# getreu/stringsext

Measured on AMD Instinct MI355X. Metric: GiB/s scanned, higher is better.
Workload: dtype u8

## Files before the change

### stringsext_amd/csrc/sx_api.cpp

```cpp
#include "sx_ctx.hpp"
#include "sx_print_core.hpp"
#include "sx_select_core.hpp"
#include "sx_selset_build.hpp"
#include "sx_selset_core.hpp"
#include "sx_selre_build.hpp"
#include "sx_selre_core.hpp"
#include "sx_extract_build.hpp"
#include "sx_extract_core.hpp"
#include "sx_seltally_build.hpp"
#include "sx_seltally_core.hpp"

using namespace sx;

struct sx_select_set {
    int device = 0;
    uint8_t* mem = nullptr;
    SelsetDevice dev{};
    sx_select_set_info info{};
};

struct sx_select_regex {
    int device = 0;
    uint8_t* mem = nullptr;
    SelreDevice dev{};
// ... 366 lines not shown
            if (d.d_pair_lut) (void)hipFree(d.d_pair_lut);
            if (d.d_wave_lut) (void)hipFree(d.d_wave_lut);
            if (d.d_wave_pairs) (void)hipFree(d.d_wave_pairs);
            if (d.d_wave_pairs2) (void)hipFree(d.d_wave_pairs2);
            for (void* q : d.d_rp) if (q) (void)hipFree(q);
            if (d.h_runs) (void)hipHostFree(d.h_runs);
            if (d.ev_runs) (void)hipEventDestroy(d.ev_runs);
            if (d.stream_w) (void)hipStreamDestroy(d.stream_w);
            if (d.h_tot) (void)hipHostFree(d.h_tot);
            if (d.h_small) (void)hipHostFree(d.h_small);
            for (hipEvent_t e : d.wave_ev) if (e) (void)hipEventDestroy(e);
            if (d.stream && d.stream != ctx->scan_stream) (void)hipStreamDestroy(d.stream);
        }
        for (int i = 0; i < 2; i++) {
            if (ctx->ing_pin[i]) (void)hipHostFree(ctx->ing_pin[i]);
            if (ctx->ing_dev[i]) (void)hipFree(ctx->ing_dev[i]);
        }
        if (ctx->copy_stream) (void)hipStreamDestroy(ctx->copy_stream);
        if (ctx->d2h_stream) (void)hipStreamDestroy(ctx->d2h_stream);
        if (ctx->scan_stream) (void)hipStreamDestroy(ctx->scan_stream);
        if (ctx->d_cache) (void)hipFree(ctx->d_cache);
        if (ctx->post_stream) (void)hipStreamDestroy(ctx->post_stream);
        if (ctx->merge_copy_stream) (void)hipStreamDestroy(ctx->merge_copy_stream);
        if (ctx->d_merge) (void)hipFree(ctx->d_merge);
        if (ctx->d_result) (void)hipFree(ctx->d_result);
        if (ctx->d_result_up) (void)hipFree(ctx->d_result_up);
        if (ctx->d_text) (void)hipFree(ctx->d_text);
        if (ctx->d_print_scratch) (void)hipFree(ctx->d_print_scratch);
        if (ctx->d_print_missions) (void)hipFree(ctx->d_print_missions);
        for (uint8_t* p : ctx->d_select) if (p) (void)hipFree(p);
        if (ctx->d_select_scratch) (void)hipFree(ctx->d_select_scratch);
        if (ctx->d_select_scratch2) (void)hipFree(ctx->d_select_scratch2);
        for (hipEvent_t e : ctx->merge_ev) if (e) (void)hipEventDestroy(e);
        if (ctx->ev_interleaved) (void)hipEventDestroy(ctx->ev_interleaved);
        if (ctx->d_input) (void)hipFree(ctx->d_input);
        if (ctx->d_scratch) (void)hipFree(ctx->d_scratch);
        if (ctx->h_pin) (void)hipHostFree(ctx->h_pin);
        if (ctx->h_pin2) (void)hipHostFree(ctx->h_pin2);
    }
    delete ctx;
}

const char* sx_last_error(const sx_ctx* ctx) { return ctx ? ctx->err.c_str() : g_create_error.c_str(); }

int sx_reset(sx_ctx* ctx) {
    if (!ctx) return SX_E_INVALID;
    for (size_t k = 0; k < ctx->missions.size(); k++) ctx->states[k].reset(ctx->missions[k]);
    ctx->shard_runs_valid = false;
    return SX_OK;
}


int sx_device_runs(sx_ctx* ctx, int mission_index, const void* device_bytes, uint64_t len, int stream_parity,
                   uint64_t min_chars, sx_run** runs, uint64_t* n_runs) {
    if (!ctx || !runs || !n_runs || mission_index < 0 || (size_t)mission_index >= ctx->missions.size()) return SX_E_INVALID;
    begin_call(ctx);
    ctx->sw.scan_warm = Switches::from_env().scan_warm;
    if (ctx->host_only) { ctx->err = "host-only context: no device scan"; return SX_E_STATE; }
    if ((uintptr_t)device_bytes & 15) { ctx->err = "device_bytes must be 16-byte aligned"; return SX_E_INVALID; }
    if (ctx->missions[(size_t)mission_index].host_sequential()) { ctx->err = "an ISO-2022-JP mission has no stage A (one sequential pass on the host)"; return SX_E_INVALID; }
    HIP_TRY(ctx, hipSetDevice(ctx->device));
    std::vector<RunList> out;
    ctx->shard_runs_valid = false;
    int rc = device_runs(ctx, { mission_index }, (const uint8_t*)device_bytes, len, { (uint32_t)(stream_parity & 1) },
                         { min_chars }, &out);
    if (rc != SX_OK) return rc;
// ... 699 lines not shown
```

### stringsext_amd/csrc/sx_ctx.hpp

```cpp
#pragma once
#include <hip/hip_runtime_api.h>
#include <stdio.h>
#include <stdlib.h>
#include <string.h>
#include <errno.h>
#include <fcntl.h>
#include <sys/mman.h>
#include <sys/stat.h>
#include <unistd.h>

#include <algorithm>
#include <atomic>
#include <chrono>
#include <condition_variable>
#include <deque>
#include <functional>
#include <mutex>
#include <string>
#include <thread>
#include <unordered_map>
#include <vector>

#include "sx_host.hpp"
#include "sx_switches.hpp"
// ... 52 lines not shown

struct ScanSlot {
    DevRun* d_recs = nullptr;
    uint32_t capacity = 0;
    uint32_t* d_counters = nullptr;
    hipEvent_t ev0 = nullptr, ev1 = nullptr;
    hipEvent_t ev_free = nullptr;
    bool free_pending = false;
    uint32_t* d_cnt = nullptr;  uint64_t cnt_cap = 0;
    uint32_t* d_grid = nullptr; uint64_t grid_cap = 0;
    DevRun* d_packed = nullptr; uint64_t packed_cap = 0;
    uint32_t region_cap = 0;
    uint64_t n_regions = 0;
    bool fused = false, fused_first = false;
};
struct MissionDev {
    hipStream_t stream = nullptr;
    hipStream_t stream_b = nullptr;
    ScanSlot slot[2];
    uint16_t* d_table = nullptr;
    uint32_t* d_pair_lut = nullptr;
    uint32_t* d_wave_pairs = nullptr;
    uint32_t* d_wave_pairs2 = nullptr;
    uint8_t* d_wave_lut = nullptr;
    sx_run* h_runs = nullptr; uint64_t h_runs_cap = 0;
    hipEvent_t ev_runs = nullptr;
    void* d_rp[12] = { nullptr, nullptr, nullptr, nullptr, nullptr, nullptr, nullptr, nullptr, nullptr, nullptr, nullptr, nullptr };
    uint64_t d_rp_cap[12] = { 0, 0, 0, 0, 0, 0, 0, 0, 0, 0, 0, 0 };
    hipStream_t stream_w = nullptr;
    uint64_t* h_tot = nullptr;
    const uint32_t* grid_of_scan = nullptr; uint32_t grid_sub = 0; const uint8_t* grid_data = nullptr; uint64_t grid_len = 0;
    uint8_t* h_small = nullptr;
    std::vector<hipEvent_t> wave_ev;
};


}

struct sx_result {
    sx::Result r;
};

struct sx_ctx {
    std::shared_ptr<sx::PinnedPool> pool = std::make_shared<sx::PinnedPool>();
    std::shared_ptr<std::atomic<uint64_t>> dev_epoch = std::make_shared<std::atomic<uint64_t>>(0);
    std::vector<sx::Mission> missions;
    std::vector<sx::ScannerState> states;
    std::vector<sx::MissionDev> dev;
    bool host_only = false;
    bool sharded_call = false, single_piece = true;
    int device = -1;
    sx_options opt{};
    sx::Switches sw;
    std::string err;
    sx_stats stats{};
    hipStream_t scan_stream = nullptr, post_stream = nullptr;
    uint8_t* d_cache = nullptr;
    uint64_t d_cache_cap = 0;
    hipStream_t merge_copy_stream = nullptr;
    hipEvent_t merge_ev[3] = { nullptr, nullptr, nullptr };
    uint8_t* d_merge = nullptr; uint64_t d_merge_cap = 0, merge_out_room = 0, merge_n_out = 0;
    uint8_t* d_result = nullptr; uint64_t d_result_cap = 0;
    uint8_t* d_result_up = nullptr; uint64_t d_result_up_cap = 0;
    uint8_t* d_text = nullptr; uint64_t d_text_cap = 0;
    uint8_t* d_print_scratch = nullptr; uint64_t d_print_scratch_cap = 0;
    uint8_t* d_print_missions = nullptr;
    uint8_t* d_select[2] = { nullptr, nullptr }; uint64_t d_select_cap[2] = { 0, 0 };
    std::shared_ptr<std::atomic<uint64_t>> select_epoch[2] = { std::make_shared<std::atomic<uint64_t>>(0), std::make_shared<std::atomic<uint64_t>>(0) };
    uint64_t select_calls = 0;
    uint8_t* d_select_scratch = nullptr; uint64_t d_select_scratch_cap = 0;
    uint8_t* d_select_scratch2 = nullptr; uint64_t d_select_scratch2_cap = 0;
    bool merge_async = false;
    bool merge_copy_pending[2] = { false, false };
    uint64_t merge_parts = 0;
    uint64_t merged_out_bytes = 0;
    double out_density = 0;
    hipEvent_t ev_interleaved = nullptr;
    std::atomic<bool> interleave_pending{ false };
    std::mutex mu;
    std::mutex err_mu;
    std::recursive_mutex grow_mu;
    void set_err(std::string text) { std::lock_guard<std::mutex> g(err_mu); err = std::move(text); }
    unsigned n_cus = 256, scan_blocks_per_cu = 8;
    hipStream_t copy_stream = nullptr;
    hipStream_t d2h_stream = nullptr;
    uint8_t* ing_pin[2] = { nullptr, nullptr };
    uint8_t* ing_dev[2] = { nullptr, nullptr };
    uint64_t ing_cap = 0, ing_dev_cap = 0;
    uint32_t region_cap = 64;
    std::vector<uint32_t> dense;
    uint8_t* d_input = nullptr;
    uint64_t d_input_cap = 0;
    uint64_t ondemand_fetches = 0;
// ... 68 lines not shown

private:
    struct Seg { uint64_t lo, hi; const uint8_t* p; };
    sx_ctx* ctx_;
    const uint8_t* d_base_;
    uint64_t len_ = 0;
    static constexpr uint64_t kBlock = 65536;
    std::unordered_map<uint64_t, std::vector<uint8_t>> blocks_;
    std::vector<Seg> segs_;
    std::deque<std::vector<uint8_t>> extra_, owned_;
    std::mutex mu_;
};

int ensure_pinned(sx_ctx* ctx, uint64_t bytes);
int ensure_pinned2(sx_ctx* ctx, uint64_t bytes);
int read_back_sync(sx_ctx* ctx, sx::MissionDev& d, hipStream_t s, void* host_dst, const void* dev_src, size_t bytes);
int read_back_async(sx_ctx* ctx, hipStream_t s, void* pinned_dst, const void* dev_src, size_t bytes);
int ensure_scratch(sx_ctx* ctx, uint64_t bytes);
int ensure_capacity(sx_ctx* ctx, ScanSlot& s, uint32_t cap);
int ensure_rp(sx_ctx* ctx, MissionDev& d, int slot, uint64_t bytes);
int ensure_cache(sx_ctx* ctx, uint64_t bytes);
unsigned usable_cpus();
unsigned replay_threads(const sx_ctx* ctx);
void begin_call(sx_ctx* ctx);

ScanParams scan_params(const sx_ctx* ctx, int mission, const ScanSlot& s, const uint8_t* d_bytes, uint64_t len,
                       uint32_t parity, uint64_t min_chars);
int stage_a_launch(sx_ctx* ctx, const std::vector<int>& which, const uint8_t* d_bytes, uint64_t len,
                   const std::vector<uint32_t>& parity, const std::vector<uint64_t>& min_chars, int si);
struct ReplayJob;
int ensure_copy_stream(sx_ctx* ctx);
bool result_stays_on_device(const sx_ctx* ctx, const ReplayJob& job);
int merge_drain(sx_ctx* ctx);
int stage_a_finish(sx_ctx* ctx, const std::vector<int>& which, const uint8_t* d_bytes, uint64_t len,
                   const std::vector<uint32_t>& parity, const std::vector<uint64_t>& min_chars, int si,
                   std::vector<RunList>* out, bool cut_into_pieces = false, const ReplayJob* wave_job = nullptr);
int device_runs(sx_ctx* ctx, const std::vector<int>& which, const uint8_t* d_bytes, uint64_t len,
                const std::vector<uint32_t>& parity, const std::vector<uint64_t>& min_chars,
                std::vector<RunList>* out);

struct ReplayJob {
    uint64_t len = 0;
    int file_id = -1;
    bool is_last = false;
    std::vector<uint64_t> lo;
    uint64_t hi = 0;
    std::vector<char> entry_exact;
    std::vector<uint64_t> consumed0, stream0;
    bool commit_state = true;
    uint32_t slice_base = 0;
    const uint8_t* d_bytes = nullptr;
};




struct PreReplayed {
    std::vector<char> done;
    std::vector<MissionFindings> per;
    std::vector<uint64_t> ends;
    explicit PreReplayed(size_t nm) : done(nm, 0), per(nm), ends(nm, 0) {}
};


constexpr int SX_WAVE_FALLBACK = 1001;
constexpr int SX_NEED_RUNS = 1002;
// ... 34 lines not shown
```

### stringsext_amd/csrc/sx_replay.cpp

```cpp
#include <stdio.h>
#include <string.h>

#include <algorithm>
#include <atomic>
#include <deque>
#include <mutex>
#include <thread>

#include "sx_host.hpp"
#include "sx_replay_core.hpp"

namespace sx {

static inline uint64_t window_start(uint64_t p, size_t W) {
    const uint64_t s = p / kInputBufLen * kInputBufLen;
    return s + (p - s) / W * W;
}
static inline uint64_t back_windows(uint64_t p, size_t W, int k) {
    uint64_t w = window_start(p, W);
    for (int i = 0; i < k && w > 0; i++) w = window_start(w - 1, W);
    return w;
}
static inline uint64_t window_end(uint64_t p, size_t W, uint64_t len) {
    const uint64_t s = p / kInputBufLen * kInputBufLen;
// ... 485 lines not shown
        while (open_end && k < v.size() && (v[k].chars_flags & kRecStartOpen) && v[k].start == r.end) {
            r.end = v[k].start + v[k].len;
            r.chars += v[k].chars_flags & kRecCharsMask;
            open_end = (v[k].chars_flags & kRecEndOpen) != 0;
            k++;
        }
        if (r.chars >= min_chars) out->push_back(r);
        i = k;
    }
}

void merge_sorted_device_runs(const DevRun* v, size_t n, uint64_t min_chars, std::vector<sx_run>* out) {
    out->clear();
    out->reserve(n / 2);
    for (size_t i = 0; i < n && v[i].start != ~0ull;) {
        sx_run r{ v[i].start, v[i].start + v[i].len, v[i].chars_flags & kRecCharsMask };
        bool open_end = (v[i].chars_flags & kRecEndOpen) != 0;
        size_t k = i + 1;
        while (open_end && k < n && v[k].start != ~0ull && (v[k].chars_flags & kRecStartOpen) && v[k].start == r.end) {
            r.end = v[k].start + v[k].len;
            r.chars += v[k].chars_flags & kRecCharsMask;
            open_end = (v[k].chars_flags & kRecEndOpen) != 0;
            k++;
        }
        if (r.chars >= min_chars) out->push_back(r);
        i = k;
    }
}

void merge_findings(std::vector<MissionFindings>& per, const std::shared_ptr<PinnedPool>& pool, Result* out, uint64_t seg_bytes) {
    out->pool = pool;
    size_t nonempty = 0, which = 0;
    for (size_t k = 0; k < per.size(); k++) if (per[k].count()) { nonempty++; which = k; }
    auto release = [&](MissionFindings& mf) { if (mf.ext.p && pool) pool->give(mf.ext); mf.ext = {}; };
    if (nonempty <= 1) {
        for (size_t k = 0; k < per.size(); k++) if (!(nonempty == 1 && k == which)) release(per[k]);
        if (nonempty == 1) {
            std::vector<MissionFindings> more = std::move(per[which].more);
            per[which].more.clear();
            out->segs.push_back(std::move(per[which])); per[which].ext = {};
            for (auto& m : more) { out->segs.push_back(std::move(m)); m.ext = {}; }
        }
        return;
    }
    size_t total = 0, bytes = 0;
    for (auto& mf : per) { total += mf.count(); bytes += mf.strings_len(); }
    std::vector<size_t> idx(per.size(), 0);
    const uint64_t seg_cap = seg_bytes ? seg_bytes : 0xFFFFFFF0ull;
    if (bytes <= seg_cap) {
        out->segs.emplace_back();
        MissionFindings& m = out->segs.back();
        m.v.reserve(total);
        m.arena.reserve(bytes);
        std::vector<size_t> base(per.size(), 0);
        for (size_t k = 0; k < per.size(); k++) { base[k] = m.arena.size(); m.arena.append(per[k].strings(), per[k].strings_len()); }
        for (;;) {
            int best = -1;
            for (size_t k = 0; k < per.size(); k++) {
                if (idx[k] >= per[k].count()) continue;
                if (best < 0) { best = (int)k; continue; }
                const sx_finding& a = per[k].data()[idx[k]];
                const sx_finding& b = per[best].data()[idx[best]];
                if (a.slice_index < b.slice_index || (a.slice_index == b.slice_index && a.position < b.position)) best = (int)k;
            }
            if (best < 0) break;
            sx_finding f = per[best].data()[idx[best]++];
            f.str_off += (uint32_t)base[best];
            m.v.push_back(f);
        }
        total = 0;
    }
    size_t done = 0;
    while (done < total) {
        out->segs.emplace_back();
        MissionFindings& m = out->segs.back();
        m.v.reserve(std::min<size_t>(total - done, 1u << 24));
        for (;;) {
            int best = -1;
            for (size_t k = 0; k < per.size(); k++) {
                if (idx[k] >= per[k].count()) continue;
                if (best < 0) { best = (int)k; continue; }
// ... 91 lines not shown
```

### stringsext_amd/csrc/sx_schedule.cpp

```cpp
#include "sx_ctx.hpp"
#include <thread>

using namespace sx;

namespace sx {

uint64_t piece_bytes(const sx_ctx* ctx, uint64_t len) {
    uint64_t piece = 0;
    bool halves = false;
    if (ctx->sw.piece_mib >= 0) piece = (uint64_t)ctx->sw.piece_mib << 20;
    else if (len >= (16ull << 30) && ctx->missions.size() >= 2 && !(ctx->opt.flags & (SX_OPT_NO_FUSED_SCAN | SX_OPT_MISSION_STREAMS | SX_OPT_RESULT_ON_DEVICE))) {
        piece = ((len / 100) * 50 + kInputBufLen - 1) / kInputBufLen * kInputBufLen;
        halves = true;
    }
    if (piece == 0 || (!halves && len < 2 * piece)) return len;
    for (const Mission& m : ctx->missions) if (m.is_dbcs()) return len;
    return piece / kInputBufLen * kInputBufLen;
}

static uint64_t seq_piece_bytes(const sx_ctx* ctx, uint64_t len) {
    uint64_t piece = 0;
    if (ctx->sw.seq_piece_kib >= 0) {
        piece = (uint64_t)ctx->sw.seq_piece_kib << 10;
        if (piece == 0) return len;
// ... 77 lines not shown
               && ctx->sw.wave_replay != 0;
    }
    bool none_scanned(const sx_ctx* ctx) const {
        if (not_scanned.size() != ctx->missions.size()) return false;
        for (char c : not_scanned) if (!c) return false;
        return true;
    }

    int fetch_base(sx_ctx* ctx) {
        base_view.reset();
        if (host_bytes) return SX_OK;
        base_view.reset(new SparseDeviceBytes(ctx, d_bytes, len));
        if (none_scanned(ctx)) return SX_OK;
        ReplayJob none;
        return download_for_replay(ctx, d_bytes, len, nullptr, base_view.get(), none);
    }
    std::vector<char> not_scanned;
    int launch(sx_ctx* ctx) {
        not_scanned.assign(ctx->missions.size(), 0);
        std::vector<int> ks; std::vector<uint32_t> par; std::vector<uint64_t> mc;
        for (int k : order) {
            if (ctx->missions[(size_t)k].host_sequential() || skip_scan(ctx, (size_t)k)) { not_scanned[(size_t)k] = 1; continue; }
            ks.push_back(k); par.push_back(parity[(size_t)k]); mc.push_back(minc[(size_t)k]);
        }
        return ks.empty() ? SX_OK : stage_a_launch(ctx, ks, d_bytes, len, par, mc, slot);
    }
    int finish_and_replay(sx_ctx* ctx, const ReplayJob& job, const std::function<int()>& after_last_finish,
                          std::vector<RunList>* runs, Result* into, uint64_t* ends) {
        const size_t nm = ctx->missions.size();
        runs->assign(nm, RunList{});
        HostBytes host_view(host_bytes ? host_bytes : (const uint8_t*)"");
        ByteView& early_view = host_bytes ? (ByteView&)host_view : (ByteView&)*base_view;
        PreReplayed pre(nm);
        if (ctx->last_runs.size() != nm) ctx->last_runs.assign(nm, 0);
        ctx->wave_off.assign(nm, 0);
        if (ctx->wave_pred.size() != nm) ctx->wave_pred.assign(nm, 0);
        std::vector<std::thread> wave_threads(nm);
        std::vector<int> wave_rc(nm, SX_OK);
        std::vector<char> threaded(nm, 0);
        struct Joiner {
            std::vector<std::thread>& t;
            ~Joiner() { for (auto& x : t) if (x.joinable()) x.join(); }
        } joiner{ wave_threads };
        const uint64_t defer_all = nm >= 2 ? (result_stays_on_device(ctx, job) ? 1 : ctx->sw.defer_min_bytes) : 0;
        if (nm >= 2 && ctx->sw.wave_threads) {
            if (ctx->wave_density.size() != nm) ctx->wave_density.assign(nm, 0.0);
            for (size_t k = 0; k < nm; k++) {
                const bool unscanned = k < not_scanned.size() && not_scanned[k];
                if (ctx->missions[k].host_sequential() || !unscanned || !wave_replay_wanted(ctx, job, k, len)) continue;
                threaded[k] = 1;
                ctx->stats.bytes_scanned += len;
                wave_threads[k] = std::thread([ctx, k, &early_view, &job, &pre, &wave_rc, defer_all]() {
                    (void)hipSetDevice(ctx->device);
                    wave_rc[k] = wave_replay_mission(ctx, k, early_view, job, &pre.per[k], &pre.ends[k], defer_all, true);
                });
            }
        }
        std::vector<size_t> order2;
        for (size_t oi = 0; oi < nm; oi++) if (!threaded[(size_t)order[oi]]) order2.push_back((size_t)order[oi]);
        for (size_t oi = 0; oi < nm; oi++) if (threaded[(size_t)order[oi]]) order2.push_back((size_t)order[oi]);
        for (size_t oi = 0; oi < nm; oi++) {
            const size_t k = order2[oi];
            std::vector<RunList> one;
            int rc = SX_OK;
            const bool unscanned = k < not_scanned.size() && not_scanned[k];
            bool replayed = false;
// ... 281 lines not shown
```

### stringsext_amd/csrc/sx_stage_b.cpp

```cpp
#include "sx_ctx.hpp"

using namespace sx;

namespace sx {

static inline uint64_t win_start_h(uint64_t p, size_t W) {
    const uint64_t s0 = p / kInputBufLen * kInputBufLen;
    return s0 + (p - s0) / W * W;
}

bool device_replay_wanted(const sx_ctx* ctx, const ReplayJob& job, size_t k, size_t n_runs) {
    if (!job.d_bytes || ctx->host_only || job.is_last || ctx->missions[k].host_sequential()) return false;
    if (ctx->opt.flags & SX_OPT_HOST_REPLAY) return false;
    if (ctx->missions[k].q > 255) return false;
    if (ctx->missions[k].c.chars_min_nb == 0) return false;
    if (ctx->sw.host_replay) return false;
    if (wave_replay_wanted(ctx, job, k, n_runs)) return true;
    return (ctx->opt.flags & SX_OPT_DEVICE_REPLAY) || ctx->sw.device_replay || n_runs >= 4096;
}

struct Slab {
    size_t i0 = 0, i1 = 0;
    bool first = true, last = true;
    int out_slot = 5;
    bool async_copy = false;
    hipEvent_t reuse_after = nullptr;
    hipEvent_t copied = nullptr;
    uint64_t lo0 = 0;
    bool entry_exact0 = false;
};
struct SlabCarry {
    uint64_t last_start = 0;
    bool last_is_entry = false, any = false;
};
constexpr int SX_RETRY_WHOLE = 1000;

static int device_replay_slab(sx_ctx* ctx, size_t k, ByteView& view, const ReplayJob& job, const RunList& runs, const Slab& sl,
                              SlabCarry& carry, MissionFindings* out, uint64_t* end_pos, uint64_t defer_min_bytes) {
    const Mission& m = ctx->missions[k];
    MissionDev& d = ctx->dev[k];
    const size_t n_all = runs.size();
    const size_t n = sl.i1 - sl.i0;
    const bool slabbed = !(sl.first && sl.last);
    const size_t W = m.window;
    const double t0 = now_ms();

    ReplayParams P{};
    bool fast_pass = false;
    bool dev_stitch = n > 0 && !ctx->sw.host_stitch;
    uint64_t* h_tot = nullptr;
    ReplayRegionOut* ro = nullptr;
    {
        int rc = ensure_pinned2(ctx, (dev_stitch ? 0 : n * sizeof(ReplayRegionOut)) + 512);
        if (rc != SX_OK) return rc;
        h_tot = (uint64_t*)ctx->h_pin2;
        ro = (ReplayRegionOut*)(ctx->h_pin2 + 384);
    }
    if (n) {
        int rc = ensure_rp(ctx, d, 0, n * sizeof(sx_run)); if (rc) return rc;
        rc = ensure_rp(ctx, d, 1, n * sizeof(ReplayRegionOut)); if (rc) return rc;
// ... 66 lines not shown
    if (dev_stitch) HIP_TRY(ctx, runs.fetch_edges(kEdgeRuns)); else HIP_TRY(ctx, runs.wait());
    const size_t head_n = runs.full() ? n_all : kEdgeRuns;
    std::deque<ReplayPart> host_parts;
    struct Seg { int host_part; size_t v0, v1; };
    std::vector<Seg> segs;
    uint64_t E = std::min(job.lo[k], job.hi);
    uint64_t last_start = carry.any ? carry.last_start : E;
    bool last_is_entry = carry.any ? carry.last_is_entry : false;
    if (job.entry_exact[k]) {
        host_parts.emplace_back();
        replay_part(m, ctx->states[k], job.consumed0[k], job.stream0[k], view, job.len, job.file_id, false, runs.data(), head_n,
                    job.lo[k], job.lo[k] + 1, true, &host_parts.back());
        if (head_n < n_all && host_parts.back().end_pos >= runs[head_n - 1].start) {
            HIP_TRY(ctx, runs.wait());
            host_parts.pop_back();
            host_parts.emplace_back();
            replay_part(m, ctx->states[k], job.consumed0[k], job.stream0[k], view, job.len, job.file_id, false, runs.data(), n_all,
                        job.lo[k], job.lo[k] + 1, true, &host_parts.back());
        }
        if (host_parts.back().regions.empty()) host_parts.pop_back();
        else { segs.push_back({ (int)host_parts.size() - 1, 0, 0 }); last_is_entry = true; E = std::max(E, host_parts.back().end_pos); }
        E = std::max(E, job.lo[k] + 1);
    }
    if (dev_stitch) {
        HIP_TRY(ctx, launch_stitch_finish(P, (const ReplayRegionOut*)d.d_rp[1], (uint8_t*)d.d_rp[2], d.d_rp[6], E,
                                          (uint64_t*)d.d_rp[3], (uint64_t*)d.d_rp[4], (uint64_t*)d.d_rp[7], ctx->d_scratch,
                                          ctx->d_scratch_cap, d.stream_b, ctx->sw.stitch_block));
        { const int rb = read_back_async(ctx, d.stream_b, h_tot, d.d_rp[7], kTotCount * 8); if (rb != SX_OK) return rb; }
    }
    SX_TL("  replay: pass 1 + stitch queued, host entry part done");
    if (n) HIP_TRY(ctx, hipStreamSynchronize(d.stream_b));
    SX_TL("  replay: pass 1 + stitch done");
    if (dev_stitch && h_tot[kTotTooLong] && slabbed) return SX_RETRY_WHOLE;
    if (dev_stitch && h_tot[kTotTooLong]) {
        dev_stitch = false;
        HIP_TRY(ctx, runs.wait());
        const uint64_t keep32 = h_tot[32], keep33 = h_tot[33];
        int rc = ensure_pinned2(ctx, n * sizeof(ReplayRegionOut) + 512);
        if (rc != SX_OK) return rc;
        h_tot = (uint64_t*)ctx->h_pin2;
        h_tot[32] = keep32; h_tot[33] = keep33;
        ro = (ReplayRegionOut*)(ctx->h_pin2 + 384);
        HIP_TRY(ctx, hipMemcpyAsync(ro, d.d_rp[1], n * sizeof(ReplayRegionOut), hipMemcpyDeviceToHost, d.stream_b));
        HIP_TRY(ctx, hipStreamSynchronize(d.stream_b));
    }
    const double t1 = now_ms();
    if (fast_pass && n) {
        std::lock_guard<std::mutex> g(ctx->mu);
        ctx->stats.fast_regions += (uint32_t)h_tot[33] - (uint32_t)h_tot[32];
        ctx->stats.general_regions += (uint32_t)h_tot[32];
    }

    std::vector<uint64_t> valid, fbase, abase;
    uint64_t nf = 0, nb = 0, n_standing = 0;
    if (dev_stitch) {
        nf = h_tot[kTotFindings]; nb = h_tot[kTotBytes]; n_standing = h_tot[kTotStanding];
        out->replay_bytes += h_tot[kTotReplayBytes];
        if (h_tot[kTotLast] != ~0ull) {
            E = std::max(E, h_tot[kTotEnd]);
            last_start = h_tot[kTotLastStart];
            last_is_entry = false;
        }
    } else {
        valid.reserve(n); fbase.reserve(n + 1); abase.reserve(n + 1);
        for (size_t i = 0; i < n; i++) {
            const uint32_t st = ro[i].status;
// ... 37 lines not shown
            else HIP_TRY(ctx, hipStreamWaitEvent(d.stream_b, sl.reuse_after, 0));
        }
        int rc = ensure_rp(ctx, d, sl.out_slot, out_bytes + 64); if (rc) return rc;
        uint8_t* d_all = (uint8_t*)d.d_rp[sl.out_slot];
        sx_finding* d_f = (sx_finding*)d_all + nfh;
        uint8_t* d_a = d_all + (nfh + nf) * sizeof(sx_finding) + nbh;
        if (dev_stitch) {
            P.str_off_base = (uint32_t)nbh;
            HIP_TRY(ctx, launch_replay_write_flagged(P, (const ReplayRegionOut*)d.d_rp[1], (const uint8_t*)d.d_rp[2],
                                                     (const uint64_t*)d.d_rp[3], (const uint64_t*)d.d_rp[4], d_f, d_a,
                                                     (nf * sizeof(sx_finding) + nb) / std::max<uint64_t>(1, n_standing), d.stream_b));
            if (nfh) {
                entry_f.assign(hf0->v.begin(), hf0->v.end());
                for (sx_finding& f : entry_f) f.slice_index += job.slice_base;
                HIP_TRY(ctx, hipMemcpyAsync(d_all, entry_f.data(), nfh * sizeof(sx_finding), hipMemcpyHostToDevice, d.stream_b));
                if (nbh) HIP_TRY(ctx, hipMemcpyAsync(d_all + (nfh + nf) * sizeof(sx_finding), hf0->arena.data(), nbh, hipMemcpyHostToDevice, d.stream_b));
            }
        } else {
            const size_t nv = valid.size();
            HIP_TRY(ctx, hipMemcpyAsync(d.d_rp[2], valid.data(), nv * 8, hipMemcpyHostToDevice, d.stream_b));
            HIP_TRY(ctx, hipMemcpyAsync(d.d_rp[3], fbase.data(), (nv + 1) * 8, hipMemcpyHostToDevice, d.stream_b));
            HIP_TRY(ctx, hipMemcpyAsync(d.d_rp[4], abase.data(), (nv + 1) * 8, hipMemcpyHostToDevice, d.stream_b));
            HIP_TRY(ctx, launch_replay_write(P, (const uint64_t*)d.d_rp[2], (const uint64_t*)d.d_rp[3],
                                             (const uint64_t*)d.d_rp[4], nv, d_f, d_a, d.stream_b));
        }
        deferred = defer_min_bytes && nf * sizeof(sx_finding) + nb >= defer_min_bytes && dev_stitch && (host_parts.empty() || entry_only);
        keep_dev = (ctx->opt.flags & SX_OPT_RESULT_ON_DEVICE) && ctx->missions.size() == 1 && defer_min_bytes == 0 && job.commit_state && !ctx->sharded_call &&
                   ctx->single_piece && sl.first && sl.last && !sl.async_copy && dev_stitch && (host_parts.empty() || entry_only);
        deferred = deferred || keep_dev;
        if (!deferred) {
            blk = ctx->pool->take(out_bytes + 64);
            if (!blk.p) { ctx->err = "hipHostMalloc failed"; return SX_E_NOMEM; }
            if (sl.async_copy) {
                HIP_TRY(ctx, hipEventRecord(ctx->merge_ev[0], d.stream_b));
                HIP_TRY(ctx, hipStreamWaitEvent(ctx->merge_copy_stream, ctx->merge_ev[0], 0));
                HIP_TRY(ctx, hipMemcpyAsync(blk.p, d_all, out_bytes, hipMemcpyDeviceToHost, ctx->merge_copy_stream));
                HIP_TRY(ctx, hipEventRecord(sl.copied, ctx->merge_copy_stream));
            } else {
                const int wgs = ctx->sw.replay_copy_wgs;
                if (wgs > 0 && out_bytes >= (1u << 20)) HIP_TRY(ctx, launch_copy_bytes(blk.p, d_all, out_bytes, (uint32_t)wgs, d.stream_b, ctx->sw.merge_copy_threads, ctx->sw.merge_copy_nt != 0));
                else HIP_TRY(ctx, hipMemcpyAsync(blk.p, d_all, out_bytes, hipMemcpyDeviceToHost, d.stream_b));
            }
        }
        SX_TL("  replay: pass 2 + copy queued (%llu bytes%s)", (unsigned long long)out_bytes, deferred ? ", stays on the device" : "");
        if (!sl.async_copy || nfh) HIP_TRY(ctx, hipStreamSynchronize(d.stream_b));
        SX_TL("  replay: pass 2 + copy done");
    }
    const double t3 = now_ms();

    if (host_parts.empty() || (entry_only && (blk.p || deferred))) {
        if (deferred) {
            out->dev_only = true; out->ext_nf = nfh + nf; out->ext_na = nbh + nb; out->dev_copy = d.d_rp[sl.out_slot];
            if (keep_dev) { out->keep_on_device = true; out->dev_epoch_ref = ctx->dev_epoch; out->dev_epoch = ctx->dev_epoch->load(); }
        }
        else if (blk.p) { out->ext = blk; out->ext_nf = nfh + nf; out->ext_na = nbh + nb; out->dev_copy = sl.async_copy ? nullptr : d.d_rp[sl.out_slot]; }
        if (hf0) out->replay_bytes += hf0->replay_bytes;
    } else {
        const sx_finding* dev_f = (const sx_finding*)blk.p;
        const char* dev_a = blk.p ? (const char*)blk.p + nf * sizeof(sx_finding) : nullptr;
        if (dev_stitch) {
            fbase.assign({ 0, nf }); abase.assign({ 0, nb });
            if (n_standing) segs.push_back({ -1, 0, 1 });
        }
        for (const Seg& g : segs) {
            if (g.host_part >= 0) {
                const MissionFindings& hf = host_parts[(size_t)g.host_part].findings;
                const uint32_t base = (uint32_t)out->arena.size();
                out->arena += hf.arena;
// ... 14 lines not shown
        uint64_t ts = win_start_h(tail, W);
        for (int t = 0; t < 3 && ts > 0; t++) ts = win_start_h(ts - 1, W);
        const uint64_t lo0 = slabbed ? sl.lo0 : job.lo[k];
        const bool exact0 = slabbed ? sl.entry_exact0 : job.entry_exact[k] != 0;
        uint64_t from = last_is_entry ? lo0 : (E > ts ? last_start : ts);
        if (from < lo0) from = lo0;
        ReplayPart fin;
        const sx_run* fr = runs.data();
        size_t fn = n_all;
        if (!runs.full()) {
            if (n_all > kEdgeRuns && runs[n_all - kEdgeRuns].start <= from) { fr = runs.data() + (n_all - kEdgeRuns); fn = kEdgeRuns; }
            else HIP_TRY(ctx, runs.wait());
        }
        replay_part(m, ctx->states[k], job.consumed0[k], job.stream0[k], view, job.len, job.file_id, false, fr, fn,
                    from, job.len, exact0 && from == lo0, &fin);
        ctx->states[k] = fin.state;
        ctx->states[k].consumed_bytes = job.consumed0[k] + job.len;
        ctx->states[k].stream_bytes = job.stream0[k] + job.len;
        E = job.len;
    }
    if (end_pos) *end_pos = std::max(E, std::min(job.hi, job.len));
    carry.last_start = last_start; carry.last_is_entry = last_is_entry; carry.any = true;
    if (ctx->sw.timing)
        fprintf(stderr, "[sx] device replay mission %zu: %zu runs, pass1+entry %.2f ms, validity %.2f ms (%zu standing, %zu host parts), "
                        "pass2+d2h %.2f ms (%llu findings), splice+state %.2f ms\n", k, n, t1 - t0, t2 - t1, (size_t)n_standing,
                host_parts.size(), t3 - t2, (unsigned long long)nf, now_ms() - t3);
    return SX_OK;
}

int ensure_copy_stream(sx_ctx* ctx) {
    if (ctx->merge_copy_stream) return SX_OK;
    HIP_TRY(ctx, hipStreamCreateWithPriority(&ctx->merge_copy_stream, hipStreamNonBlocking, 0));
    for (hipEvent_t& e : ctx->merge_ev) HIP_TRY(ctx, hipEventCreateWithFlags(&e, hipEventDisableTiming));
    return SX_OK;
}

int device_replay_mission(sx_ctx* ctx, size_t k, ByteView& view, const ReplayJob& job, const RunList& runs,
                          MissionFindings* out, uint64_t* end_pos, uint64_t defer_min_bytes) {
    const size_t n = runs.size();
    MissionDev& d = ctx->dev[k];
    if (wave_replay_wanted(ctx, job, k, n)) {
        const int rc = wave_replay_mission(ctx, k, view, job, out, end_pos, defer_min_bytes);
        if (rc != SX_WAVE_FALLBACK) return rc;
        if (k < ctx->wave_off.size()) ctx->wave_off[k] = 1;
        if (k < ctx->wave_pred.size()) ctx->wave_pred[k] = 0;
    }
    if (runs.skipped) return SX_NEED_RUNS;
    size_t K = 1;
    const bool can = ctx->missions.size() == 1 && runs.on_device && !ctx->sw.host_stitch && defer_min_bytes == 0;
    const bool keep_dev_wanted = (ctx->opt.flags & SX_OPT_RESULT_ON_DEVICE) && ctx->missions.size() == 1 && defer_min_bytes == 0 && job.commit_state && !ctx->sharded_call && ctx->single_piece;
    if (can && n >= (1u << 20) && !keep_dev_wanted) K = 3;
    if (ctx->sw.slabs) { K = (size_t)ctx->sw.slabs; if (!can || n < 8 * K) K = 1; }
    std::vector<uint64_t> idx{ 0 }, his{ 0 };
    if (K > 1) {
        int rc = ensure_copy_stream(ctx); if (rc != SX_OK) return rc;
        rc = ensure_scratch(ctx, 4096); if (rc != SX_OK) return rc;
        rc = ensure_pinned2(ctx, 4096); if (rc != SX_OK) return rc;
        ReplayParams P{};
        P.runs = runs.dev_ptr; P.n_runs = n; P.W = (uint32_t)ctx->missions[k].window; P.grep_char = ctx->missions[k].c.grep_char;
        uint64_t* d_cut = (uint64_t*)ctx->d_scratch;
        HIP_TRY(ctx, launch_slab_cuts(P, (uint32_t)K, d_cut, d_cut + 64, d.stream_b));
        { const int rb = read_back_async(ctx, d.stream_b, ctx->h_pin2, d_cut, 128 * 8); if (rb != SX_OK) return rb; }
        HIP_TRY(ctx, hipStreamSynchronize(d.stream_b));
        const uint64_t* h = (const uint64_t*)ctx->h_pin2;
        for (size_t j = 1; j < K; j++)
            if (h[j - 1] > idx.back() && h[j - 1] < n && h[64 + j - 1] < job.hi) { idx.push_back(h[j - 1]); his.push_back(h[64 + j - 1]); }
    }
    idx.push_back(n);
    const size_t ns = idx.size() - 1;
    if (ns > 1) {
        std::vector<MissionFindings> got;
        SlabCarry carry;
        hipEvent_t copied[2] = { ctx->merge_ev[1], ctx->merge_ev[2] };
        uint64_t e_prev = 0;
        int rc = SX_OK;
        for (size_t j = 0; j < ns && rc == SX_OK; j++) {
            ReplayJob sj = job;
            sj.hi = j + 1 < ns ? std::min(job.hi, his[j + 1]) : job.hi;
            if (j > 0) { sj.lo[k] = std::max(job.lo[k], e_prev); sj.entry_exact[k] = 0; }
            sj.commit_state = job.commit_state && j + 1 == ns;
            Slab sl;
            sl.i0 = idx[j]; sl.i1 = idx[j + 1]; sl.first = j == 0; sl.last = j + 1 == ns;
            sl.out_slot = (j & 1) ? 8 : 5; sl.async_copy = true;
            sl.reuse_after = j >= 2 ? copied[j & 1] : nullptr; sl.copied = copied[j & 1];
            sl.lo0 = job.lo[k]; sl.entry_exact0 = job.entry_exact[k] != 0;
            MissionFindings mf;
            uint64_t e_now = 0;
            rc = device_replay_slab(ctx, k, view, sj, runs, sl, carry, &mf, &e_now, 0);
            e_prev = std::max(e_prev, e_now);
            if (rc == SX_OK) {
                out->replay_bytes += mf.replay_bytes; mf.replay_bytes = 0;
                if (mf.count()) got.push_back(std::move(mf));
            } else if (mf.ext.p) got.push_back(std::move(mf));
        }
        (void)hipStreamSynchronize(ctx->merge_copy_stream);
        (void)hipStreamSynchronize(d.stream_b);
        if (rc == SX_OK) {
            const uint64_t rb = out->replay_bytes;
            if (!got.empty()) {
                *out = std::move(got[0]);
                for (size_t j = 1; j < got.size(); j++) out->more.push_back(std::move(got[j]));
            }
            out->replay_bytes = rb;
            if (end_pos) *end_pos = e_prev;
            return SX_OK;
        }
        for (auto& g : got) if (g.ext.p) ctx->pool->give(g.ext);
        out->replay_bytes = 0;
        if (rc != SX_RETRY_WHOLE) return rc;
    }
    Slab sl;
    sl.i1 = n;
    SlabCarry carry;
    return device_replay_slab(ctx, k, view, job, runs, sl, carry, out, end_pos, defer_min_bytes);
}

static int fetch_deferred(sx_ctx* ctx, MissionFindings& mf) {
    if (!mf.dev_only) return SX_OK;
    const size_t bytes = mf.ext_nf * sizeof(sx_finding) + mf.ext_na;
    PinnedPool::Block blk = ctx->pool->take(bytes + 64);
    if (!blk.p) { ctx->err = "hipHostMalloc failed"; return SX_E_NOMEM; }
    HIP_TRY(ctx, hipMemcpyAsync(blk.p, mf.dev_copy, bytes, hipMemcpyDeviceToHost, ctx->post_stream));
    HIP_TRY(ctx, hipStreamSynchronize(ctx->post_stream));
    mf.ext = blk; mf.dev_only = false;
    return SX_OK;
}

bool result_stays_on_device(const sx_ctx* ctx, const ReplayJob& job) {
    return (ctx->opt.flags & SX_OPT_RESULT_ON_DEVICE) && ctx->missions.size() >= 2 && merge_part_can_pack(1, (int)ctx->missions.size()) && !ctx->host_only &&
           job.d_bytes && job.commit_state && !ctx->sharded_call && ctx->single_piece && !ctx->sw.host_merge;
}

static int upload_host_lists(sx_ctx* ctx, std::vector<MissionFindings>& per, std::vector<char>& uploaded) {
    uint64_t need = 0;
    for (auto& mf : per) {
        if (!mf.count() || mf.dev_copy) continue;
        if (!mf.more.empty() || mf.packed) return SX_E_NOMEM;
        need += (mf.count() * sizeof(sx_finding) + mf.strings_len() + 255) & ~(uint64_t)255;
    }
    if (!need) return SX_OK;
    if (ctx->d_result_up_cap < need) {
        if (ctx->d_result_up) HIP_TRY(ctx, hipFree(ctx->d_result_up));
        ctx->d_result_up = nullptr; ctx->d_result_up_cap = 0;
        if (hipMalloc((void**)&ctx->d_result_up, need) != hipSuccess) { (void)hipGetLastError(); ctx->d_result_up = nullptr; return SX_E_NOMEM; }
        ctx->d_result_up_cap = need;
    }
    PinnedPool::Block blk = ctx->pool->take(need);
    if (!blk.p) return SX_E_NOMEM;
    uint64_t at = 0;
    for (size_t k = 0; k < per.size(); k++) {
        MissionFindings& mf = per[k];
        if (!mf.count() || mf.dev_copy) continue;
        const uint64_t fb = mf.count() * sizeof(sx_finding);
        memcpy((uint8_t*)blk.p + at, mf.data(), fb);
        memcpy((uint8_t*)blk.p + at + fb, mf.strings(), mf.strings_len());
        mf.dev_copy = ctx->d_result_up + at; uploaded[k] = 1;
        at += (fb + mf.strings_len() + 255) & ~(uint64_t)255;
    }
    hipError_t e = hipMemcpyAsync(ctx->d_result_up, blk.p, need, hipMemcpyHostToDevice, ctx->post_stream);
    if (e == hipSuccess) e = hipStreamSynchronize(ctx->post_stream);
    ctx->pool->give(blk);
    if (e != hipSuccess) {
        for (size_t k = 0; k < per.size(); k++) if (uploaded[k]) { per[k].dev_copy = nullptr; uploaded[k] = 0; }
        HIP_TRY(ctx, e);
    }
    return SX_OK;
}

int merge_drain(sx_ctx* ctx) {
    std::lock_guard<std::recursive_mutex> g(ctx->grow_mu);
    if (ctx->post_stream) HIP_TRY(ctx, hipStreamSynchronize(ctx->post_stream));
    if (ctx->merge_copy_stream) HIP_TRY(ctx, hipStreamSynchronize(ctx->merge_copy_stream));
    ctx->merge_copy_pending[0] = ctx->merge_copy_pending[1] = false;
    ctx->interleave_pending = false;
    return SX_OK;
}

static int device_merge(sx_ctx* ctx, const ReplayJob& job, std::vector<MissionFindings>& per, Result* into) {
    const size_t nm = per.size();
    size_t with = 0, on_dev = 0, deferred = 0;
    uint64_t total = 0, bytes = 0;
    bool same_origin = true;
    for (size_t k = 0; k < nm; k++) {
        if (!per[k].count()) continue;
        with++;
        if ((per[k].ext.p || per[k].dev_only) && per[k].dev_copy) on_dev++;
        if (per[k].dev_only) deferred++;
        total += per[k].count(); bytes += per[k].strings_len();
        same_origin = same_origin && job.consumed0[k] == job.consumed0[0];
    }
    std::vector<char> uploaded(nm, 0);
    auto give_up = [&]() -> int {
        for (size_t k = 0; k < nm; k++) if (uploaded[k]) { per[k].dev_copy = nullptr; uploaded[k] = 0; }
        for (auto& mf : per) { if (mf.keep_on_device) continue; int rc = fetch_deferred(ctx, mf); if (rc != SX_OK) return rc; }
        return SX_OK;
    };
    bool keep = result_stays_on_device(ctx, job) && total > 0 && same_origin;
    if (keep && on_dev != with) {
        const int rc = upload_host_lists(ctx, per, uploaded);
        if (rc == SX_E_NOMEM) keep = false;
        else if (rc != SX_OK) return rc;
        else on_dev = with;
    }
    auto host_way_ok = [&]() { return with >= 2 && on_dev == with && same_origin && total >= 4096 && !ctx->sw.host_merge; };
    if (!keep && !host_way_ok()) return give_up();
    const double tm0 = now_ms();
// ... 178 lines not shown
static int host_sequential_mission(sx_ctx* ctx, size_t k, ByteView& bytes, const ReplayJob& job, MissionFindings* out) {
    const Mission& m = ctx->missions[k];
    ScannerState st = ctx->states[k];
    if (bytes.all_on_host() || !job.d_bytes) {
        replay_exact_windows(m, st, job.consumed0[k], job.stream0[k], bytes, job.len, job.file_id, 0, job.len, out, job.is_last);
    } else {
        struct Piece : ByteView {
            std::vector<uint8_t> buf; uint64_t base = 0;
            const uint8_t* span(uint64_t off, size_t, size_t*) override { return buf.data() + (off - base); }
        } piece;
        const uint64_t step = 64ull << 20;
        for (uint64_t at = 0; at < job.len; at += step) {
            const uint64_t n = std::min(step, job.len - at);
            piece.buf.resize(n); piece.base = at;
            HIP_TRY(ctx, hipMemcpy(piece.buf.data(), job.d_bytes + at, n, hipMemcpyDeviceToHost));
            replay_exact_windows(m, st, job.consumed0[k], job.stream0[k], piece, job.len, job.file_id, at, at + n, out, job.is_last);
        }
    }
    out->replay_bytes += job.len;
    if (job.slice_base) for (auto& f : out->v) f.slice_index += job.slice_base;
    if (job.commit_state) {
        st.consumed_bytes = job.consumed0[k] + job.len;
        st.stream_bytes = job.stream0[k] + job.len;
        ctx->states[k] = st;
    }
    return SX_OK;
}

int replay_all(sx_ctx* ctx, ByteView& bytes, const ReplayJob& job, const std::vector<RunList>& runs,
               Result* into, uint64_t* end_pos, PreReplayed* pre) {
    const double t0 = now_ms();
    const size_t nm = ctx->missions.size();
    const unsigned nthreads = replay_threads(ctx);
    std::vector<std::vector<uint64_t>> bounds(nm);
    std::vector<std::vector<ReplayPart>> parts(nm);
    std::vector<std::pair<size_t, size_t>> tasks;
    std::vector<char> on_device(nm, 0);
    uint64_t host_runs = 0;
    for (size_t k = 0; k < nm; k++)
        on_device[k] = (pre && pre->done[k]) ? 2 : ctx->missions[k].host_sequential() ? 3 : (device_replay_wanted(ctx, job, k, runs[k].size()) ? 1 : 0);
    for (size_t k = 0; k < nm; k++) {
        if (on_device[k]) continue;
        HIP_TRY(ctx, runs[k].wait());
        unsigned want_parts = (unsigned)std::min<uint64_t>(nthreads, std::max<uint64_t>(1, runs[k].size() / 512));
        if (ctx->missions[k].c.chars_min_nb == 0) want_parts = 1;
        host_runs += runs[k].size();
        replay_plan_range(std::min(job.lo[k], job.hi), job.hi, want_parts, &bounds[k]);
        parts[k].resize(bounds[k].size() - 1);
        for (size_t p = 0; p + 1 < bounds[k].size(); p++) tasks.emplace_back(k, p);
    }
    std::atomic<size_t> next{ 0 };
    std::vector<double> task_ms(tasks.size(), 0.0);
    auto worker = [&]() {
        for (;;) {
            const size_t t = next.fetch_add(1);
            if (t >= tasks.size()) break;
            const size_t k = tasks[t].first, p = tasks[t].second;
            const double tt0 = now_ms();
            replay_part(ctx->missions[k], ctx->states[k], job.consumed0[k], job.stream0[k], bytes, job.len, job.file_id,
                        job.is_last, runs[k].data(), runs[k].size(), bounds[k][p], bounds[k][p + 1],
                        p == 0 && job.entry_exact[k], &parts[k][p]);
            task_ms[t] = now_ms() - tt0;
        }
    };
    const size_t nw = host_runs < 2048 ? 1 : std::min<size_t>(nthreads, tasks.size());
    if (nw <= 1) worker();
// ... 4 lines not shown
    }
    const double t_parts = now_ms();
    std::vector<MissionFindings> per(nm);
    std::vector<uint64_t> ends(nm, 0);
    for (size_t k = 0; k < nm; k++) {
        if (on_device[k] == 2) { per[k] = std::move(pre->per[k]); pre->per[k].ext = {}; ends[k] = pre->ends[k]; }
        else if (on_device[k] == 3) {
            int rc = host_sequential_mission(ctx, k, bytes, job, &per[k]);
            if (rc != SX_OK) return rc;
            ends[k] = job.len;
        } else if (on_device[k]) {
            int rc = device_replay_mission(ctx, k, bytes, job, runs[k], &per[k], &ends[k], 0);
            if (rc != SX_OK) return rc;
        }
    }
    auto stitch = [&](size_t k) {
        if (on_device[k]) return;
        ScannerState st = ctx->states[k];
        replay_stitch(ctx->missions[k], st, job.consumed0[k], job.stream0[k], bytes, job.len, job.file_id, job.is_last,
                      runs[k].data(), runs[k].size(), parts[k], &per[k], nthreads, &ends[k]);
        if (job.commit_state) ctx->states[k] = st;
        if (job.slice_base) for (auto& f : per[k].v) f.slice_index += job.slice_base;
    };
    if (nm == 1) stitch(0);
    else {
        std::vector<std::thread> th;
        for (size_t k = 0; k < nm; k++) th.emplace_back(stitch, k);
        for (auto& t : th) t.join();
    }
    if (end_pos) for (size_t k = 0; k < nm; k++) end_pos[k] = ends[k];
    const double t_stitch = now_ms();
    SX_TL("replay_all: host parts + stitch done");
    const size_t count_before = into->count();
    {
        int rc = device_merge(ctx, job, per, into);
        if (rc != SX_OK) return rc;
    }
    SX_TL("replay_all: device_merge done");
    merge_findings(per, ctx->pool, into, ctx->sw.host_merge_seg_bytes);
    SX_TL("replay_all: merge_findings done");
    if (ctx->sw.timing) {
        double mx = 0, sum = 0;
        for (double v : task_ms) { sum += v; mx = std::max(mx, v); }
        fprintf(stderr, "[sx] replay: parts %.2f ms (%zu tasks, %zu workers; task sum %.1f max %.1f ms), stitch %.2f ms, merge %.2f ms, "
                        "on-demand fetches so far %llu\n", t_parts - t0, tasks.size(), nw, sum, mx, t_stitch - t_parts,
                now_ms() - t_stitch, (unsigned long long)ctx->ondemand_fetches);
    }
    for (auto& mf : per) ctx->stats.replay_bytes += mf.replay_bytes;
    ctx->stats.findings += into->count() - count_before;
    ctx->stats.replay_ms += now_ms() - t0;
    return SX_OK;
}

ReplayJob whole_chunk_job(sx_ctx* ctx, uint64_t len, int file_id, bool is_last) {
    ReplayJob j;
    const size_t nm = ctx->missions.size();
    j.len = len; j.file_id = file_id; j.is_last = is_last; j.hi = len;
    j.lo.assign(nm, 0); j.entry_exact.assign(nm, 1);
    for (size_t k = 0; k < nm; k++) { j.consumed0.push_back(ctx->states[k].consumed_bytes); j.stream0.push_back(ctx->states[k].stream_bytes); }
    return j;
}


int download_for_replay(sx_ctx* ctx, const uint8_t* d_bytes, uint64_t len,
                               const std::vector<RunList>* runs_opt, SparseDeviceBytes* view,
                               const ReplayJob& job, const std::vector<char>* skip, bool* used_base) {
// ... 75 lines not shown
```

Measured before the change: 3994.

## Enable slabbed device replay beside host-replayed missions with deferred copy drain

Device replay is now split into slabs even when other missions exist, provided those missions replay on the host. It uses 2 slabs, sized against a per-mission output estimate taken from the previous call. The final D2H slab copies are no longer synchronized inside the mission. They drain just before the merge, so the copies overlap host replay and stitch of the other missions. merge_findings gains a block-aware k-way merge for the multi-block results, and slabs abort to a whole replay if their output would exceed the deferred budget. This adds complexity and a risk of retries that redo the work.

```diff
diff --git a/stringsext_amd/csrc/sx_api.cpp b/stringsext_amd/csrc/sx_api.cpp
--- a/stringsext_amd/csrc/sx_api.cpp
+++ b/stringsext_amd/csrc/sx_api.cpp
@@ -422,6 +422,7 @@
         if (ctx->d_select_scratch) (void)hipFree(ctx->d_select_scratch);
         if (ctx->d_select_scratch2) (void)hipFree(ctx->d_select_scratch2);
         for (hipEvent_t e : ctx->merge_ev) if (e) (void)hipEventDestroy(e);
+        for (hipEvent_t e : ctx->slab_ev) if (e) (void)hipEventDestroy(e);
         if (ctx->ev_interleaved) (void)hipEventDestroy(ctx->ev_interleaved);
         if (ctx->d_input) (void)hipFree(ctx->d_input);
         if (ctx->d_scratch) (void)hipFree(ctx->d_scratch);
diff --git a/stringsext_amd/csrc/sx_ctx.hpp b/stringsext_amd/csrc/sx_ctx.hpp
--- a/stringsext_amd/csrc/sx_ctx.hpp
+++ b/stringsext_amd/csrc/sx_ctx.hpp
@@ -108,6 +108,7 @@
     const uint32_t* grid_of_scan = nullptr; uint32_t grid_sub = 0; const uint8_t* grid_data = nullptr; uint64_t grid_len = 0;
     uint8_t* h_small = nullptr;
     std::vector<hipEvent_t> wave_ev;
+    uint64_t last_out_runs = 0, last_out_bytes = 0;
 };
 
 
@@ -135,6 +136,8 @@
     uint64_t d_cache_cap = 0;
     hipStream_t merge_copy_stream = nullptr;
     hipEvent_t merge_ev[3] = { nullptr, nullptr, nullptr };
+    hipEvent_t slab_ev[3] = { nullptr, nullptr, nullptr };
+    std::atomic<bool> slab_copy_pending{ false };
     uint8_t* d_merge = nullptr; uint64_t d_merge_cap = 0, merge_out_room = 0, merge_n_out = 0;
     uint8_t* d_result = nullptr; uint64_t d_result_cap = 0;
     uint8_t* d_result_up = nullptr; uint64_t d_result_up_cap = 0;
@@ -269,6 +272,7 @@
 int ensure_copy_stream(sx_ctx* ctx);
 bool result_stays_on_device(const sx_ctx* ctx, const ReplayJob& job);
 int merge_drain(sx_ctx* ctx);
+int slab_copy_drain(sx_ctx* ctx);
 int stage_a_finish(sx_ctx* ctx, const std::vector<int>& which, const uint8_t* d_bytes, uint64_t len,
                    const std::vector<uint32_t>& parity, const std::vector<uint64_t>& min_chars, int si,
                    std::vector<RunList>* out, bool cut_into_pieces = false, const ReplayJob* wave_job = nullptr);
diff --git a/stringsext_amd/csrc/sx_replay.cpp b/stringsext_amd/csrc/sx_replay.cpp
--- a/stringsext_amd/csrc/sx_replay.cpp
+++ b/stringsext_amd/csrc/sx_replay.cpp
@@ -541,7 +541,11 @@
     out->pool = pool;
     size_t nonempty = 0, which = 0;
     for (size_t k = 0; k < per.size(); k++) if (per[k].count()) { nonempty++; which = k; }
-    auto release = [&](MissionFindings& mf) { if (mf.ext.p && pool) pool->give(mf.ext); mf.ext = {}; };
+    auto release = [&](MissionFindings& mf) {
+        if (mf.ext.p && pool) pool->give(mf.ext);
+        mf.ext = {};
+        for (auto& x : mf.more) { if (x.ext.p && pool) pool->give(x.ext); x.ext = {}; }
+    };
     if (nonempty <= 1) {
         for (size_t k = 0; k < per.size(); k++) if (!(nonempty == 1 && k == which)) release(per[k]);
         if (nonempty == 1) {
@@ -552,10 +556,61 @@
         }
         return;
     }
+    const uint64_t seg_cap = seg_bytes ? seg_bytes : 0xFFFFFFF0ull;
+    bool in_blocks = false;
+    for (auto& mf : per) in_blocks = in_blocks || !mf.more.empty();
+    if (in_blocks) {
+        struct Cursor { std::vector<const MissionFindings*> blocks; size_t b = 0, i = 0; };
+        std::vector<Cursor> cur(per.size());
+        for (size_t k = 0; k < per.size(); k++) {
+            if (per[k].count()) cur[k].blocks.push_back(&per[k]);
+            for (auto& x : per[k].more) if (x.count()) cur[k].blocks.push_back(&x);
+        }
+        auto head = [](Cursor& c) -> const sx_finding* {
+            while (c.b < c.blocks.size() && c.i >= c.blocks[c.b]->count()) { c.b++; c.i = 0; }
+            return c.b < c.blocks.size() ? c.blocks[c.b]->data() + c.i : nullptr;
+        };
+        bool open = false;
+        const char* run_src = nullptr;
+        uint64_t run_off = 0, run_len = 0;
+        auto flush = [&]() {
+            if (run_len) out->segs.back().arena.append(run_src + run_off, run_len);
+            run_src = nullptr; run_len = 0;
+        };
+        for (;;) {
+            int best = -1;
+            const sx_finding* bf = nullptr;
+            for (size_t k = 0; k < per.size(); k++) {
+                const sx_finding* f = head(cur[k]);
+                if (!f) continue;
+                if (best < 0 || f->slice_index < bf->slice_index || (f->slice_index == bf->slice_index && f->position < bf->position)) { best = (int)k; bf = f; }
+            }
+            if (best < 0) break;
+            Cursor& c = cur[(size_t)best];
+            const MissionFindings& src = *c.blocks[c.b];
+            const bool next_block = c.i == 0 && c.b > 0;
+            if (!open || next_block || out->segs.back().arena.size() + run_len + bf->str_len > seg_cap) {
+                flush();
+                out->segs.emplace_back();
+                out->segs.back().v.reserve(src.count() - c.i + 64);
+                out->segs.back().arena.reserve(std::min<uint64_t>(seg_cap, src.strings_len() + 4096));
+                open = true;
+            }
+            MissionFindings& m = out->segs.back();
+            if (run_src != src.strings() || bf->str_off != run_off + run_len) { flush(); run_src = src.strings(); run_off = bf->str_off; }
+            sx_finding f = *bf;
+            f.str_off = (uint32_t)(m.arena.size() + run_len);
+            run_len += bf->str_len;
+            m.v.push_back(f);
+            c.i++;
+        }
+        flush();
+        for (auto& mf : per) { release(mf); mf.more.clear(); }
+        return;
+    }
     size_t total = 0, bytes = 0;
     for (auto& mf : per) { total += mf.count(); bytes += mf.strings_len(); }
     std::vector<size_t> idx(per.size(), 0);
-    const uint64_t seg_cap = seg_bytes ? seg_bytes : 0xFFFFFFF0ull;
     if (bytes <= seg_cap) {
         out->segs.emplace_back();
         MissionFindings& m = out->segs.back();
diff --git a/stringsext_amd/csrc/sx_schedule.cpp b/stringsext_amd/csrc/sx_schedule.cpp
--- a/stringsext_amd/csrc/sx_schedule.cpp
+++ b/stringsext_amd/csrc/sx_schedule.cpp
@@ -133,6 +133,7 @@
         HostBytes host_view(host_bytes ? host_bytes : (const uint8_t*)"");
         ByteView& early_view = host_bytes ? (ByteView&)host_view : (ByteView&)*base_view;
         PreReplayed pre(nm);
+        struct SlabDrain { sx_ctx* ctx; ~SlabDrain() { (void)slab_copy_drain(ctx); } } slab_drain{ ctx };
         if (ctx->last_runs.size() != nm) ctx->last_runs.assign(nm, 0);
         ctx->wave_off.assign(nm, 0);
         if (ctx->wave_pred.size() != nm) ctx->wave_pred.assign(nm, 0);
diff --git a/stringsext_amd/csrc/sx_stage_b.cpp b/stringsext_amd/csrc/sx_stage_b.cpp
--- a/stringsext_amd/csrc/sx_stage_b.cpp
+++ b/stringsext_amd/csrc/sx_stage_b.cpp
@@ -26,6 +26,8 @@
     bool async_copy = false;
     hipEvent_t reuse_after = nullptr;
     hipEvent_t copied = nullptr;
+    hipEvent_t written = nullptr;
+    uint64_t out_budget = 0;
     uint64_t lo0 = 0;
     bool entry_exact0 = false;
 };
@@ -158,6 +160,7 @@
     if (n) HIP_TRY(ctx, hipStreamSynchronize(d.stream_b));
     SX_TL("  replay: pass 1 + stitch done");
     if (dev_stitch && h_tot[kTotTooLong] && slabbed) return SX_RETRY_WHOLE;
+    if (dev_stitch && slabbed && sl.out_budget && h_tot[kTotFindings] * sizeof(sx_finding) + h_tot[kTotBytes] >= sl.out_budget) return SX_RETRY_WHOLE;
     if (dev_stitch && h_tot[kTotTooLong]) {
         dev_stitch = false;
         HIP_TRY(ctx, runs.wait());
@@ -261,8 +264,9 @@
             blk = ctx->pool->take(out_bytes + 64);
             if (!blk.p) { ctx->err = "hipHostMalloc failed"; return SX_E_NOMEM; }
             if (sl.async_copy) {
-                HIP_TRY(ctx, hipEventRecord(ctx->merge_ev[0], d.stream_b));
-                HIP_TRY(ctx, hipStreamWaitEvent(ctx->merge_copy_stream, ctx->merge_ev[0], 0));
+                ctx->slab_copy_pending = true;
+                HIP_TRY(ctx, hipEventRecord(sl.written, d.stream_b));
+                HIP_TRY(ctx, hipStreamWaitEvent(ctx->merge_copy_stream, sl.written, 0));
                 HIP_TRY(ctx, hipMemcpyAsync(blk.p, d_all, out_bytes, hipMemcpyDeviceToHost, ctx->merge_copy_stream));
                 HIP_TRY(ctx, hipEventRecord(sl.copied, ctx->merge_copy_stream));
             } else {
@@ -343,7 +347,22 @@
     if (ctx->merge_copy_stream) return SX_OK;
     HIP_TRY(ctx, hipStreamCreateWithPriority(&ctx->merge_copy_stream, hipStreamNonBlocking, 0));
     for (hipEvent_t& e : ctx->merge_ev) HIP_TRY(ctx, hipEventCreateWithFlags(&e, hipEventDisableTiming));
+    for (hipEvent_t& e : ctx->slab_ev) HIP_TRY(ctx, hipEventCreateWithFlags(&e, hipEventDisableTiming));
     return SX_OK;
+}
+
+int slab_copy_drain(sx_ctx* ctx) {
+    if (!ctx->slab_copy_pending.exchange(false)) return SX_OK;
+    HIP_TRY(ctx, hipStreamSynchronize(ctx->merge_copy_stream));
+    return SX_OK;
+}
+
+static bool slabs_next_to_others(const sx_ctx* ctx, size_t k, const ReplayJob& job) {
+    if (ctx->missions.size() < 2 || (ctx->opt.flags & SX_OPT_RESULT_ON_DEVICE) || ctx->merge_async || ctx->sharded_call) return false;
+    if (ctx->last_runs.size() != ctx->missions.size()) return false;
+    for (size_t o = 0; o < ctx->missions.size(); o++)
+        if (o != k && (ctx->missions[o].host_sequential() || device_replay_wanted(ctx, job, o, ctx->last_runs[o]))) return false;
+    return true;
 }
 
 int device_replay_mission(sx_ctx* ctx, size_t k, ByteView& view, const ReplayJob& job, const RunList& runs,
@@ -357,10 +376,20 @@
         if (k < ctx->wave_pred.size()) ctx->wave_pred[k] = 0;
     }
     if (runs.skipped) return SX_NEED_RUNS;
+    auto note_output = [&]() {
+        uint64_t bytes = out->count() * sizeof(sx_finding) + out->strings_len();
+        for (const MissionFindings& m : out->more) bytes += m.count() * sizeof(sx_finding) + m.strings_len();
+        d.last_out_runs = n; d.last_out_bytes = bytes;
+    };
     size_t K = 1;
-    const bool can = ctx->missions.size() == 1 && runs.on_device && !ctx->sw.host_stitch && defer_min_bytes == 0;
+    const bool alone = ctx->missions.size() == 1 && defer_min_bytes == 0;
+    const bool beside = !alone && slabs_next_to_others(ctx, k, job);
+    const bool can = (alone || beside) && runs.on_device && !ctx->sw.host_stitch;
     const bool keep_dev_wanted = (ctx->opt.flags & SX_OPT_RESULT_ON_DEVICE) && ctx->missions.size() == 1 && defer_min_bytes == 0 && job.commit_state && !ctx->sharded_call && ctx->single_piece;
-    if (can && n >= (1u << 20) && !keep_dev_wanted) K = 3;
+    if (can && n >= (1u << 20) && !keep_dev_wanted) {
+        K = beside ? 2 : 3;
+        if (beside && (!d.last_out_runs || (defer_min_bytes && 2.0 * (double)n * (double)d.last_out_bytes / (double)d.last_out_runs >= (double)defer_min_bytes))) K = 1;
+    }
     if (ctx->sw.slabs) { K = (size_t)ctx->sw.slabs; if (!can || n < 8 * K) K = 1; }
     std::vector<uint64_t> idx{ 0 }, his{ 0 };
     if (K > 1) {
@@ -382,8 +411,10 @@
     if (ns > 1) {
         std::vector<MissionFindings> got;
         SlabCarry carry;
-        hipEvent_t copied[2] = { ctx->merge_ev[1], ctx->merge_ev[2] };
-        uint64_t e_prev = 0;
+        hipEvent_t copied[2] = { ctx->slab_ev[1], ctx->slab_ev[2] };
+        uint64_t e_prev = 0, written = 0;
+        uint64_t fast0 = 0, general0 = 0;
+        { std::lock_guard<std::mutex> g(ctx->mu); fast0 = ctx->stats.fast_regions; general0 = ctx->stats.general_regions; }
         int rc = SX_OK;
         for (size_t j = 0; j < ns && rc == SX_OK; j++) {
             ReplayJob sj = job;
@@ -393,19 +424,22 @@
             Slab sl;
             sl.i0 = idx[j]; sl.i1 = idx[j + 1]; sl.first = j == 0; sl.last = j + 1 == ns;
             sl.out_slot = (j & 1) ? 8 : 5; sl.async_copy = true;
-            sl.reuse_after = j >= 2 ? copied[j & 1] : nullptr; sl.copied = copied[j & 1];
+            sl.reuse_after = j >= 2 ? copied[j & 1] : nullptr; sl.copied = copied[j & 1]; sl.written = ctx->slab_ev[0];
             sl.lo0 = job.lo[k]; sl.entry_exact0 = job.entry_exact[k] != 0;
+            if (defer_min_bytes) {
+                if (written >= defer_min_bytes) { rc = SX_RETRY_WHOLE; break; }
+                sl.out_budget = defer_min_bytes - written;
+            }
             MissionFindings mf;
             uint64_t e_now = 0;
             rc = device_replay_slab(ctx, k, view, sj, runs, sl, carry, &mf, &e_now, 0);
             e_prev = std::max(e_prev, e_now);
             if (rc == SX_OK) {
                 out->replay_bytes += mf.replay_bytes; mf.replay_bytes = 0;
+                written += mf.count() * sizeof(sx_finding) + mf.strings_len();
                 if (mf.count()) got.push_back(std::move(mf));
             } else if (mf.ext.p) got.push_back(std::move(mf));
         }
-        (void)hipStreamSynchronize(ctx->merge_copy_stream);
-        (void)hipStreamSynchronize(d.stream_b);
         if (rc == SX_OK) {
             const uint64_t rb = out->replay_bytes;
             if (!got.empty()) {
@@ -414,16 +448,23 @@
             }
             out->replay_bytes = rb;
             if (end_pos) *end_pos = e_prev;
+            note_output();
             return SX_OK;
         }
+        (void)hipStreamSynchronize(ctx->merge_copy_stream);
+        (void)hipStreamSynchronize(d.stream_b);
+        ctx->slab_copy_pending = false;
         for (auto& g : got) if (g.ext.p) ctx->pool->give(g.ext);
         out->replay_bytes = 0;
         if (rc != SX_RETRY_WHOLE) return rc;
+        { std::lock_guard<std::mutex> g(ctx->mu); ctx->stats.fast_regions = fast0; ctx->stats.general_regions = general0; }
     }
     Slab sl;
     sl.i1 = n;
     SlabCarry carry;
-    return device_replay_slab(ctx, k, view, job, runs, sl, carry, out, end_pos, defer_min_bytes);
+    const int rc = device_replay_slab(ctx, k, view, job, runs, sl, carry, out, end_pos, defer_min_bytes);
+    if (rc == SX_OK) note_output();
+    return rc;
 }
 
 static int fetch_deferred(sx_ctx* ctx, MissionFindings& mf) {
@@ -483,6 +524,7 @@
     if (ctx->post_stream) HIP_TRY(ctx, hipStreamSynchronize(ctx->post_stream));
     if (ctx->merge_copy_stream) HIP_TRY(ctx, hipStreamSynchronize(ctx->merge_copy_stream));
     ctx->merge_copy_pending[0] = ctx->merge_copy_pending[1] = false;
+    ctx->slab_copy_pending = false;
     ctx->interleave_pending = false;
     return SX_OK;
 }
@@ -727,6 +769,7 @@
     const double t0 = now_ms();
     const size_t nm = ctx->missions.size();
     const unsigned nthreads = replay_threads(ctx);
+    struct SlabDrain { sx_ctx* ctx; ~SlabDrain() { (void)slab_copy_drain(ctx); } } slab_drain{ ctx };
     std::vector<std::vector<uint64_t>> bounds(nm);
     std::vector<std::vector<ReplayPart>> parts(nm);
     std::vector<std::pair<size_t, size_t>> tasks;
@@ -797,6 +840,11 @@
     const double t_stitch = now_ms();
     SX_TL("replay_all: host parts + stitch done");
     const size_t count_before = into->count();
+    {
+        int rc = slab_copy_drain(ctx);
+        if (rc != SX_OK) return rc;
+    }
+    SX_TL("replay_all: slab copies done");
     {
         int rc = device_merge(ctx, job, per, into);
         if (rc != SX_OK) return rc;
```

Result: faster. 4112 (median of 6 runs) (+3.0%).
